# lvjiahui/DRT

Hardware: AMD Instinct MI355X
Metric: M camera-rays/s (forward+backward) on 50k-tri mesh, 72 views (higher is better)
Workload: dtype f32 traversal + f64 shading/gradients; 1 GPU; horse_vh.ply x4 (1 midpoint subdivision) = 50248 tris / 25126 verts, 72 turntable views, 1024x1024 rays/view, LBVH rebuilt every step, forward+ray_loss+backward+all-reduce+SGD; targets=horse_scan.ply, mode=dropin, hip_graph=False, outputs_recycled=True, ray_binding=True, views_per_gpu=72, views_per_call=72

## Files before the change

### drt_amd/csrc/drt_raster.hip

```cpp
#include "drt_device.h"

__global__ void __launch_bounds__(64) k_fit_views(const double* __restrict__ origin, const double* __restrict__ dir, int w, int h,
                                                  ViewModel* __restrict__ views) {
    __shared__ ViewModel vm;
    const int64_t base = (int64_t)blockIdx.x * w * h;
    if (threadIdx.x == 0) {
        const int64_t i00 = base, iW0 = base + (w - 1), i0H = base + (int64_t)(h - 1) * w, iWH = i0H + (w - 1);
        if (fit_view_model(load_d3(origin, i00), load_d3(dir, i00), load_d3(dir, iW0), load_d3(dir, i0H), load_d3(dir, iWH),
                           (double)(w - 1), (double)(h - 1), vm))
            vm.ok = 1;
    }
    __syncthreads();
    bool good = vm.ok != 0;
    if (good) {
        const int sx = (int)(threadIdx.x & 7), sy = (int)(threadIdx.x >> 3);
        const int x = (int)(((int64_t)(w - 1) * sx) / 7), y = (int)(((int64_t)(h - 1) * sy) / 7);
        const int64_t i = base + (int64_t)y * w + x;
        good = view_verify(vm, load_d3(origin, i), load_d3(dir, i), (double)x, (double)y);
    }
    const bool all_good = __ballot(good) == ~0ull;
    if (threadIdx.x == 0) {
        vm.ok = all_good ? 1 : 0;
        vm.all = vm.ok;
        views[blockIdx.x] = vm;
    }
}

__device__ __forceinline__ uint32_t canary_hash(uint32_t a, uint32_t b, uint32_t c) {
    uint32_t h = a * 0x9E3779B1u ^ (b + 0x7F4A7C15u) * 0x85EBCA6Bu ^ (c + 0x165667B1u) * 0xC2B2AE35u;
    h ^= h >> 15; h *= 0x2C1B3C6Du; h ^= h >> 12; h *= 0x297A2D39u; h ^= h >> 15;
    return h;
}
__global__ void __launch_bounds__(64) k_check_views(const double* __restrict__ origin, const double* __restrict__ dir, int w, int h,
                                                    ViewModel* __restrict__ cache, ViewModel* __restrict__ views, unsigned salt, unsigned* __restrict__ salt_ctr) {
    __shared__ ViewModel vm;
    __shared__ unsigned s_ctr;
    const int64_t base = (int64_t)blockIdx.x * w * h;
    if (threadIdx.x == 0) {
        vm = cache[blockIdx.x];
        s_ctr = salt_ctr ? __hip_atomic_load(salt_ctr, __ATOMIC_RELAXED, __HIP_MEMORY_SCOPE_AGENT) : 0u;
        if (salt_ctr && blockIdx.x == 0) atomicAdd(salt_ctr, 1u);
    }
    __syncthreads();
    if (salt) salt = (salt ^ (s_ctr * 0x9E3779B1u)) | 1u;
    const bool trusted = vm.ok && vm.all;
    const int sx = (int)(threadIdx.x & 7), sy = (int)(threadIdx.x >> 3);
    const int x = (int)(((int64_t)(w - 1) * sx) / 7), y = (int)(((int64_t)(h - 1) * sy) / 7);
    const int64_t i = base + (int64_t)y * w + x;
    bool good = trusted && view_verify(vm, load_d3(origin, i), load_d3(dir, i), (double)x, (double)y);
    if (good && salt) {
        const uint32_t hx = canary_hash(salt, blockIdx.x, threadIdx.x), hy = canary_hash(salt ^ 0xA5A5A5A5u, threadIdx.x, blockIdx.x);
        const int cx = (int)(((uint64_t)hx * (uint64_t)w) >> 32), cy = (int)(((uint64_t)hy * (uint64_t)h) >> 32);
        const int64_t ci = base + (int64_t)cy * w + cx;
        good = view_verify(vm, load_d3(origin, ci), load_d3(dir, ci), (double)cx, (double)cy);
    }
    if (__ballot(good) == ~0ull) {
        if (threadIdx.x == 0) views[blockIdx.x] = vm;
        return;
    }
    __syncthreads();
    if (threadIdx.x == 0) {
        const int64_t i00 = base, iW0 = base + (w - 1), i0H = base + (int64_t)(h - 1) * w, iWH = i0H + (w - 1);
        if (fit_view_model(load_d3(origin, i00), load_d3(dir, i00), load_d3(dir, iW0), load_d3(dir, i0H), load_d3(dir, iWH),
                           (double)(w - 1), (double)(h - 1), vm))
            vm.ok = 1;
    }
    __syncthreads();
    good = vm.ok != 0 && view_verify(vm, load_d3(origin, i), load_d3(dir, i), (double)x, (double)y);
    const bool all_good = __ballot(good) == ~0ull;
    if (threadIdx.x == 0) {
        vm.ok = all_good ? 1 : 0;
        vm.all = 0;
        views[blockIdx.x] = vm;
        if (trusted) { cache[blockIdx.x].ok = 0; cache[blockIdx.x].all = 0; }
    }
}

__device__ __forceinline__ void raster_test(const TriRec& t, f3 o32, const double* __restrict__ dir, int64_t i, int64_t slot,
                                            unsigned long long* __restrict__ zbuf, uint32_t* __restrict__ zmask) {
    const f3 d32 = to_f32(load_d3(dir, i));
    float tt;
    if (!tri_hit_mt(o32, d32, f3{t.v0x, t.v0y, t.v0z}, f3{t.e1x, t.e1y, t.e1z}, f3{t.e2x, t.e2y, t.e2z}, tt)) return;
    const unsigned long long key = raster_key(tt, t.face);
    if (key >= zbuf[slot]) return;
    if (!hit_point_in_box(o32, d32, tt, f3{t.v0x, t.v0y, t.v0z}, f3{t.e1x, t.e1y, t.e1z}, f3{t.e2x, t.e2y, t.e2z}, t.margin)) return;
    atomicMin(&zbuf[slot], key);
    const uint32_t bit = 1u << ((i >> 6) & 31);
    if (!(zmask[i >> 11] & bit)) atomicOr(&zmask[i >> 11], bit);
}

struct BigItem { int32_t view, tri, x0, y0, nx, ny; };

struct RasterLane {
    TriRec tri;
    int32_t x0, y0, nx, end;
};

__global__ void __launch_bounds__(256) k_raster(const TriRec* __restrict__ tris, int n_tris, ViewModel* views,
                                                const double* __restrict__ dir, int w, int h,
                                                unsigned long long* __restrict__ zbuf, uint32_t* __restrict__ zmask,
                                                BigItem* __restrict__ big, unsigned* big_count, unsigned big_cap, int pass) {
    __shared__ RasterLane s_lane[256];
    const int view = blockIdx.y;
    const ViewModel vm = views[view];
    if (!vm.ok) return;
    const int k = blockIdx.x * 256 + threadIdx.x;
    const int lane = threadIdx.x & 63, wbase = threadIdx.x & ~63;
    const d3 o{vm.o[0], vm.o[1], vm.o[2]};
    const f3 o32 = to_f32(o);
    int count = 0;
    RasterLane me;
    me.x0 = me.y0 = 0; me.nx = 1;
    if (k < n_tris) {
        me.tri = tris[k];
        if ((pass == 1) == tri_faces_away(o32, me.tri)) {
            const PixelBox box = project_tri_box(vm, o32, me.tri, w, h);
            if (box.unsafe) {
                __hip_atomic_store(&views[view].ok, 0, __ATOMIC_RELAXED, __HIP_MEMORY_SCOPE_AGENT);
            } else if (box.x0 <= box.x1 && box.y0 <= box.y1) {
                me.x0 = box.x0; me.y0 = box.y0; me.nx = box.x1 - box.x0 + 1;
                const int ny = box.y1 - box.y0 + 1;
                const int64_t cnt = (int64_t)me.nx * ny;
                if (cnt > kRasterMaxPerLane) {
                    const int rows_per = max(1, kRasterBandPixels / me.nx), n_bands = (ny + rows_per - 1) / rows_per;
                    const unsigned slot = atomicAdd(big_count, (unsigned)n_bands);
                    if (slot <= big_cap && (unsigned)n_bands <= big_cap - slot) {
                        for (int b = 0; b < n_bands; ++b)
                            big[slot + b] = BigItem{view, k, me.x0, me.y0 + b * rows_per, me.nx, min(rows_per, ny - b * rows_per)};
                    } else {
                        __hip_atomic_store(&views[view].ok, 0, __ATOMIC_RELAXED, __HIP_MEMORY_SCOPE_AGENT);
                        for (unsigned q = slot; q < big_cap; ++q) big[q] = BigItem{view, k, 0, 0, 0, 0};
                    }
                } else {
                    count = (int)cnt;
                }
            }
        }
    }
    int end = count;
    for (int off = 1; off < 64; off <<= 1) {
        const int v = __shfl_up(end, off);
        if (lane >= off) end += v;
    }
    const int total = __shfl(end, 63);
    if (total == 0) return;
    me.end = end;
    s_lane[threadIdx.x] = me;
    __builtin_amdgcn_wave_barrier();
    const int64_t base = (int64_t)view * w * h;
    for (int item0 = 0; item0 < total; item0 += 64) {
        const int item = item0 + lane;
        if (item >= total) break;
        int lo = 0, hi = 63;
        while (lo < hi) {
            const int mid = (lo + hi) >> 1;
            if (s_lane[wbase + mid].end > item) hi = mid; else lo = mid + 1;
        }
        const RasterLane& ow = s_lane[wbase + lo];
        const int local = item - (lo == 0 ? 0 : s_lane[wbase + lo - 1].end);
        const int row = (int)(((float)local + 0.5f) / (float)ow.nx);
        const int x = ow.x0 + (local - row * ow.nx), y = ow.y0 + row;
        raster_test(ow.tri, o32, dir, base + (int64_t)y * w + x, raster_slot((unsigned)x, (unsigned)(view * h + y), (unsigned)w), zbuf, zmask);
    }
}

__global__ void __launch_bounds__(256) k_raster_big(const TriRec* __restrict__ tris, const ViewModel* __restrict__ views,
                                                    const double* __restrict__ dir, int w, int h,
                                                    unsigned long long* __restrict__ zbuf, uint32_t* __restrict__ zmask,
                                                    const BigItem* __restrict__ big, const unsigned* __restrict__ big_count, unsigned big_cap) {
    const unsigned n = min(*big_count, big_cap);
    const unsigned n_waves = gridDim.x * 4u;
    const int lane = threadIdx.x & 63;
    for (unsigned e = __builtin_amdgcn_readfirstlane(blockIdx.x * 4u + (threadIdx.x >> 6)); e < n; e += n_waves) {
        const BigItem it = big[e];
        const ViewModel& vm = views[it.view];
        const TriRec t = tris[it.tri];
        const f3 o32 = to_f32(d3{vm.o[0], vm.o[1], vm.o[2]});
        const int64_t base = (int64_t)it.view * w * h;
        const int cnt = it.nx * it.ny;
        for (int p = lane; p < cnt; p += 64) {
            const int row = (int)(((float)p + 0.5f) / (float)it.nx);
            int y = it.y0 + row, x = it.x0 + (p - row * it.nx);
            if (x >= it.x0 + it.nx) { x -= it.nx; ++y; } else if (x < it.x0) { x += it.nx; --y; }
            raster_test(t, o32, dir, base + (int64_t)y * w + x, raster_slot((unsigned)x, (unsigned)(it.view * h + y), (unsigned)w), zbuf, zmask);
        }
    }
}

__global__ void k_fill_u64(unsigned long long* __restrict__ p, int64_t n, unsigned long long v) {
    for (int64_t i = blockIdx.x * (int64_t)blockDim.x + threadIdx.x; i < n; i += (int64_t)gridDim.x * blockDim.x) p[i] = v;
}

int ensure_raster(drt_scene* s, drt_scene::Sub& w, int64_t n_rays, int n_views, hipStream_t st) {
    if (n_rays > w.z_cap) {
        (void)hipFree(w.zbuf); (void)hipFree(w.zmask);
        w.zbuf = nullptr; w.zmask = nullptr; w.z_cap = 0;
        const int64_t words = (n_rays + 2047) / 2048 + 1;
        HIP_TRY(hipMalloc(&w.zbuf, sizeof(unsigned long long) * n_rays));
        HIP_TRY(hipMalloc(&w.zmask, sizeof(uint32_t) * words));
        k_fill_u64<<<4 * s->n_cu, 256, 0, st>>>(w.zbuf, n_rays, kRasterEmpty);
        HIP_TRY(hipMemsetAsync(w.zmask, 0, sizeof(uint32_t) * words, st));
        w.z_cap = n_rays;
    }
    if (n_views > w.vm_cap) {
        (void)hipFree(w.vmodel); w.vmodel = nullptr; w.vm_cap = 0;
        HIP_TRY(hipMalloc(&w.vmodel, sizeof(ViewModel) * n_views));
        w.vm_cap = n_views;
    }
    if (!w.big) {
        HIP_TRY(hipMalloc(&w.big, sizeof(BigItem) * drt_scene::kBigCap));
        HIP_TRY(hipMalloc(&w.big_count, sizeof(unsigned)));
    }
    return DRT_OK;
}

int launch_raster(drt_scene* s, drt_scene::Sub& w, hipStream_t st, const double* d_origin, const double* d_dir, int n_views, int iw, int ih,
                  ViewModel* trusted) {
    const int n = (int)s->n_faces;
    HIP_TRY(hipMemsetAsync(w.big_count, 0, sizeof(unsigned), st));
    if (trusted) k_check_views<<<n_views, 64, 0, st>>>(d_origin, d_dir, iw, ih, trusted, w.vmodel,
                                                        s->grid_canary ? (++s->canary_salt ? s->canary_salt : ++s->canary_salt) : 0u,
                                                        s->vcount + 3);
    else k_fit_views<<<n_views, 64, 0, st>>>(d_origin, d_dir, iw, ih, w.vmodel);
    if (n > 0) {
        for (int pass = 0; pass < 2; ++pass) {
            k_raster<<<dim3((n + 255) / 256, n_views), 256, 0, st>>>(s->tris_flat, n, w.vmodel, d_dir, iw, ih, w.zbuf, w.zmask,
                                                                      reinterpret_cast<BigItem*>(w.big), w.big_count, drt_scene::kBigCap, pass);
            if (pass == 0) {
                k_raster_big<<<8 * s->n_cu, 256, 0, st>>>(s->tris_flat, w.vmodel, d_dir, iw, ih, w.zbuf, w.zmask,
                                                           reinterpret_cast<const BigItem*>(w.big), w.big_count, drt_scene::kBigCap);
                HIP_TRY(hipMemsetAsync(w.big_count, 0, sizeof(unsigned), st));
            }
        }
        k_raster_big<<<8 * s->n_cu, 256, 0, st>>>(s->tris_flat, w.vmodel, d_dir, iw, ih, w.zbuf, w.zmask,
                                                   reinterpret_cast<const BigItem*>(w.big), w.big_count, drt_scene::kBigCap);
    }
    HIP_TRY(hipGetLastError());
    return DRT_OK;
}
```

Measured before the change: 44300 M camera-rays/s.

## Make triangle raster kernel persistent with wave-strided runs over views and triangles

Replaces the 2D grid of one block per (triangle chunk, view) with a persistent grid of 8 blocks per CU. Each wave loops over 64-triangle runs across all views, reloading the view model only when the view changes and keeping it as wave-uniform float values. This is meant to cut launch and block scheduling overhead and to avoid re-reading the full double-precision ViewModel per block. The projection matrix is now rounded to float before the per-triangle box projection, which can change conservative pixel bounds. The kernel also sets a minimum occupancy in launch bounds, which may force register spilling.

```diff
diff --git a/drt_amd/csrc/drt_raster.hip b/drt_amd/csrc/drt_raster.hip
--- a/drt_amd/csrc/drt_raster.hip
+++ b/drt_amd/csrc/drt_raster.hip
@@ -96,71 +96,84 @@
     int32_t x0, y0, nx, end;
 };
 
-__global__ void __launch_bounds__(256) k_raster(const TriRec* __restrict__ tris, int n_tris, ViewModel* views,
-                                                const double* __restrict__ dir, int w, int h,
-                                                unsigned long long* __restrict__ zbuf, uint32_t* __restrict__ zmask,
-                                                BigItem* __restrict__ big, unsigned* big_count, unsigned big_cap, int pass) {
+__device__ __forceinline__ float wave_uniform(float v) { return __int_as_float(__builtin_amdgcn_readfirstlane(__float_as_int(v))); }
+
+__global__ void __launch_bounds__(256, 8) k_raster(const TriRec* __restrict__ tris, int n_tris, ViewModel* views, int n_views,
+                                                   const double* __restrict__ dir, int w, int h,
+                                                   unsigned long long* __restrict__ zbuf, uint32_t* __restrict__ zmask,
+                                                   BigItem* __restrict__ big, unsigned* big_count, unsigned big_cap, int pass) {
     __shared__ RasterLane s_lane[256];
-    const int view = blockIdx.y;
-    const ViewModel vm = views[view];
-    if (!vm.ok) return;
-    const int k = blockIdx.x * 256 + threadIdx.x;
-    const int lane = threadIdx.x & 63, wbase = threadIdx.x & ~63;
-    const d3 o{vm.o[0], vm.o[1], vm.o[2]};
-    const f3 o32 = to_f32(o);
-    int count = 0;
-    RasterLane me;
-    me.x0 = me.y0 = 0; me.nx = 1;
-    if (k < n_tris) {
-        me.tri = tris[k];
-        if ((pass == 1) == tri_faces_away(o32, me.tri)) {
-            const PixelBox box = project_tri_box(vm, o32, me.tri, w, h);
-            if (box.unsafe) {
-                __hip_atomic_store(&views[view].ok, 0, __ATOMIC_RELAXED, __HIP_MEMORY_SCOPE_AGENT);
-            } else if (box.x0 <= box.x1 && box.y0 <= box.y1) {
-                me.x0 = box.x0; me.y0 = box.y0; me.nx = box.x1 - box.x0 + 1;
-                const int ny = box.y1 - box.y0 + 1;
-                const int64_t cnt = (int64_t)me.nx * ny;
-                if (cnt > kRasterMaxPerLane) {
-                    const int rows_per = max(1, kRasterBandPixels / me.nx), n_bands = (ny + rows_per - 1) / rows_per;
-                    const unsigned slot = atomicAdd(big_count, (unsigned)n_bands);
-                    if (slot <= big_cap && (unsigned)n_bands <= big_cap - slot) {
-                        for (int b = 0; b < n_bands; ++b)
-                            big[slot + b] = BigItem{view, k, me.x0, me.y0 + b * rows_per, me.nx, min(rows_per, ny - b * rows_per)};
+    const int lane = threadIdx.x & 63;
+    RasterLane* const wl = s_lane + (threadIdx.x & ~63);
+    const unsigned n_waves = gridDim.x * 4u, wave = __builtin_amdgcn_readfirstlane(blockIdx.x * 4u + (threadIdx.x >> 6));
+    const unsigned runs_per_view = ((unsigned)n_tris + 63u) / 64u, n_runs = runs_per_view * (unsigned)n_views;
+    int cur_view = -1;
+    float minv32[9] = {};
+    f3 o32{0.0f, 0.0f, 0.0f};
+    for (unsigned run = wave; run < n_runs; run += n_waves) {
+        const int view = (int)(run / runs_per_view);
+        const int k = (int)(run - (unsigned)view * runs_per_view) * 64 + lane;
+        if (!__hip_atomic_load(&views[view].ok, __ATOMIC_RELAXED, __HIP_MEMORY_SCOPE_AGENT)) continue;
+        if (view != cur_view) {
+            cur_view = view;
+            for (int q = 0; q < 9; ++q) minv32[q] = wave_uniform((float)views[view].minv[q]);
+            o32 = f3{wave_uniform((float)views[view].o[0]), wave_uniform((float)views[view].o[1]), wave_uniform((float)views[view].o[2])};
+        }
+        int count = 0;
+        __builtin_amdgcn_wave_barrier();
+        if (k < n_tris) {
+            const TriRec tri = tris[k];
+            if ((pass == 1) == tri_faces_away(o32, tri)) {
+                ViewModel vm;
+                for (int q = 0; q < 9; ++q) vm.minv[q] = (double)minv32[q];
+                const PixelBox box = project_tri_box(vm, o32, tri, w, h);
+                if (box.unsafe) {
+                    __hip_atomic_store(&views[view].ok, 0, __ATOMIC_RELAXED, __HIP_MEMORY_SCOPE_AGENT);
+                } else if (box.x0 <= box.x1 && box.y0 <= box.y1) {
+                    const int nx = box.x1 - box.x0 + 1, ny = box.y1 - box.y0 + 1;
+                    const int64_t cnt = (int64_t)nx * ny;
+                    if (cnt > kRasterMaxPerLane) {
+                        const int rows_per = max(1, kRasterBandPixels / nx), n_bands = (ny + rows_per - 1) / rows_per;
+                        const unsigned slot = atomicAdd(big_count, (unsigned)n_bands);
+                        if (slot <= big_cap && (unsigned)n_bands <= big_cap - slot) {
+                            for (int b = 0; b < n_bands; ++b)
+                                big[slot + b] = BigItem{view, k, box.x0, box.y0 + b * rows_per, nx, min(rows_per, ny - b * rows_per)};
+                        } else {
+                            __hip_atomic_store(&views[view].ok, 0, __ATOMIC_RELAXED, __HIP_MEMORY_SCOPE_AGENT);
+                            for (unsigned q = slot; q < big_cap; ++q) big[q] = BigItem{view, k, 0, 0, 0, 0};
+                        }
                     } else {
-                        __hip_atomic_store(&views[view].ok, 0, __ATOMIC_RELAXED, __HIP_MEMORY_SCOPE_AGENT);
-                        for (unsigned q = slot; q < big_cap; ++q) big[q] = BigItem{view, k, 0, 0, 0, 0};
+                        count = (int)cnt;
+                        wl[lane].tri = tri;
+                        wl[lane].x0 = box.x0; wl[lane].y0 = box.y0; wl[lane].nx = nx;
                     }
-                } else {
-                    count = (int)cnt;
                 }
             }
         }
-    }
-    int end = count;
-    for (int off = 1; off < 64; off <<= 1) {
-        const int v = __shfl_up(end, off);
-        if (lane >= off) end += v;
-    }
-    const int total = __shfl(end, 63);
-    if (total == 0) return;
-    me.end = end;
-    s_lane[threadIdx.x] = me;
-    __builtin_amdgcn_wave_barrier();
-    const int64_t base = (int64_t)view * w * h;
-    for (int item0 = 0; item0 < total; item0 += 64) {
-        const int item = item0 + lane;
-        if (item >= total) break;
-        int lo = 0, hi = 63;
-        while (lo < hi) {
-            const int mid = (lo + hi) >> 1;
-            if (s_lane[wbase + mid].end > item) hi = mid; else lo = mid + 1;
-        }
-        const RasterLane& ow = s_lane[wbase + lo];
-        const int local = item - (lo == 0 ? 0 : s_lane[wbase + lo - 1].end);
-        const int row = (int)(((float)local + 0.5f) / (float)ow.nx);
-        const int x = ow.x0 + (local - row * ow.nx), y = ow.y0 + row;
-        raster_test(ow.tri, o32, dir, base + (int64_t)y * w + x, raster_slot((unsigned)x, (unsigned)(view * h + y), (unsigned)w), zbuf, zmask);
+        int end = count;
+        for (int off = 1; off < 64; off <<= 1) {
+            const int v = __shfl_up(end, off);
+            if (lane >= off) end += v;
+        }
+        const int total = __builtin_amdgcn_readlane(end, 63);
+        if (total == 0) continue;
+        wl[lane].end = end;
+        __builtin_amdgcn_wave_barrier();
+        const int64_t base = (int64_t)view * w * h;
+        for (int item0 = 0; item0 < total; item0 += 64) {
+            const int item = item0 + lane;
+            if (item >= total) break;
+            int lo = 0, hi = 63;
+            while (lo < hi) {
+                const int mid = (lo + hi) >> 1;
+                if (wl[mid].end > item) hi = mid; else lo = mid + 1;
+            }
+            const RasterLane& ow = wl[lo];
+            const int local = item - (lo == 0 ? 0 : wl[lo - 1].end);
+            const int row = (int)(((float)local + 0.5f) / (float)ow.nx);
+            const int x = ow.x0 + (local - row * ow.nx), y = ow.y0 + row;
+            raster_test(ow.tri, o32, dir, base + (int64_t)y * w + x, raster_slot((unsigned)x, (unsigned)(view * h + y), (unsigned)w), zbuf, zmask);
+        }
     }
 }
 
@@ -224,7 +237,7 @@
     else k_fit_views<<<n_views, 64, 0, st>>>(d_origin, d_dir, iw, ih, w.vmodel);
     if (n > 0) {
         for (int pass = 0; pass < 2; ++pass) {
-            k_raster<<<dim3((n + 255) / 256, n_views), 256, 0, st>>>(s->tris_flat, n, w.vmodel, d_dir, iw, ih, w.zbuf, w.zmask,
+            k_raster<<<8 * s->n_cu, 256, 0, st>>>(s->tris_flat, n, w.vmodel, n_views, d_dir, iw, ih, w.zbuf, w.zmask,
                                                                       reinterpret_cast<BigItem*>(w.big), w.big_count, drt_scene::kBigCap, pass);
             if (pass == 0) {
                 k_raster_big<<<8 * s->n_cu, 256, 0, st>>>(s->tris_flat, w.vmodel, d_dir, iw, ih, w.zbuf, w.zmask,
```

Measured after the change: 45320 M camera-rays/s, median of 6. +2.3%, better.
